# sebastianffx/stainlib

Hardware: AMD Instinct MI355X
Metric: 1024x1024 H&E tiles/sec normalized (Macenko) (higher is better)
Workload: dtype f32; 1 GPU; configs[1]: batch of 512 tiles 1024x1024x3 uint8 per GPU, Macenko transform (fit once outside the timed region), tiles resident in HBM; tiles_per_gpu=512, failed_tiles=0

## Files before the change

### stainlib_amd/csrc/stats_twosweep.hpp

```cpp
#pragma once
#include "stats_cube.hpp"

namespace sl {

constexpr double kClusterDeff = 2.0;
constexpr double kTiltZ = 5.0;
constexpr double kTiltZ4 = 4.0;
constexpr double kTsMinTau = 2e-4, kTsMaxTau = 0.05;
constexpr int kTsBackoff = 3;
constexpr double kTsAutoMaxTau = 6e-3;
constexpr int kTsMinTissue = 256;
constexpr int kTsMaxSharePct = 40;
constexpr int kTsFn = 9;
constexpr int kTsTabFloats = kTsFn * 3 * 32;

enum { kTsDirect = 1, kTsOff = 0, kTsNoEstimate = -1, kTsShare = -2, kTsPlane = -3, kTsBracket = -4, kTsLists = -5 };

struct TwoSweep {
    int ok;
    int dense;
    int pad_;
    int why;
    double Vd[6];
    double nd[3];
    double gH[3], gL[3];
    double kappa1, kappa2;
    double tau;
    float lo0, hi1;
    float fgH[3], fgL[3];
    float fn[3], fk1;
    float W[2][3], kt[2];
    float eps[2], zeta[2], thr[2];
};

struct __attribute__((packed, aligned(1))) U32U { uint32_t v; };
__device__ __forceinline__ uint32_t cluster_word(const uint8_t* src, int P, uint32_t wl, uint32_t b) {
    const uint32_t i = b / (uint32_t)kClusterPx, j = b % (uint32_t)kClusterPx;
    const uint32_t h = sample_hash(i);
    const uint32_t line = i * wl + __umulhi(h << 8, wl);
    uint32_t px = (line * 128u + 2u) / 3u + (h >> 28) % 3u + (uint32_t)kClusterStep * j;
    px = px < (uint32_t)(P - 2) ? px : (uint32_t)(P - 2);
    return ((SL_GLOBAL const U32U*)(as_global(src) + 3 * (size_t)px))->v & 0xffffffu;
}
__device__ __forceinline__ void ts_box(const double* Vd, const double* nd, double tau, const float* box, double lam, int lane, MergedConc& mk) {
    const bool finite = (box[0] > -INFINITY) & (box[1] < INFINITY) & (box[2] > -INFINITY) & (box[3] < INFINITY);
    const int g = lane % 9, var = (lane / 9) % 5;
    const int i0 = g % 3, i1 = g / 3;
    double u1[3], u2[3];
#pragma unroll
    for (int c = 0; c < 3; ++c) { u1[c] = Vd[2 * c]; u2[c] = Vd[2 * c + 1]; }
    {
        const double s = (var == 1 || var == 3) ? tau : ((var == 2 || var == 4) ? -tau : 0.0);
        const bool first = var == 1 || var == 2;
        double a[3], b[3];
#pragma unroll
        for (int c = 0; c < 3; ++c) { a[c] = (first ? u1[c] : u2[c]) + s * nd[c]; b[c] = first ? u2[c] : u1[c]; }
        const double na = 1.0 / sqrt(a[0] * a[0] + a[1] * a[1] + a[2] * a[2]);
#pragma unroll
        for (int c = 0; c < 3; ++c) a[c] *= na;
        const double ab = a[0] * b[0] + a[1] * b[1] + a[2] * b[2];
#pragma unroll
        for (int c = 0; c < 3; ++c) b[c] -= ab * a[c];
        const double nb = 1.0 / sqrt(b[0] * b[0] + b[1] * b[1] + b[2] * b[2]);
#pragma unroll
        for (int c = 0; c < 3; ++c) { b[c] *= nb; u1[c] = first ? a[c] : b[c]; u2[c] = first ? b[c] : a[c]; }
    }
    double U[6];
#pragma unroll
    for (int c = 0; c < 3; ++c) { U[2 * c] = u1[c]; U[2 * c + 1] = u2[c]; }
    const double m0 = 0.5 * ((double)box[0] + (double)box[1]), r0 = 0.5 * ((double)box[1] - (double)box[0]);
    const double m1 = 0.5 * ((double)box[2] + (double)box[3]), r1 = 0.5 * ((double)box[3] - (double)box[2]);
    const double p0 = finite ? m0 + (double)(i0 - 1) * r0 : -0.25;
    const double p1 = finite ? m1 + (double)(i1 - 1) * r1 : 0.25;
    double M[6];
    stain_matrix_from_phi(U, angle_of_pseudo(p0), angle_of_pseudo(p1), M);
    LassoD A, C;
    lasso_affine_d(M, lam, A);
#pragma unroll
    for (int i = 0; i < 2; ++i) {
#pragma unroll
        for (int c = 0; c < 3; ++c) C.W[i][c] = __shfl(A.W[i][c], 4, 64);
        C.k[i] = __shfl(A.k[i], 4, 64);
    }
    C.g12 = __shfl(A.g12, 4, 64);
    double Mc[6];
#pragma unroll
    for (int i = 0; i < 6; ++i) Mc[i] = __shfl(M[i], 4, 64);
    double T[2][2], r[2];
    relate_affine(A, C, T, r);
    double e0 = fmax(fabs(T[0][0] - 1.0), fabs(T[0][1])), e1 = fmax(fabs(T[1][1] - 1.0), fabs(T[1][0]));
    double q0 = fabs(r[0]), q1 = fabs(r[1]);
    double z0 = fabs(A.W[0][0] * nd[0] + A.W[0][1] * nd[1] + A.W[0][2] * nd[2]), z1 = fabs(A.W[1][0] * nd[0] + A.W[1][1] * nd[1] + A.W[1][2] * nd[2]);
    const bool live = lane < 45;
    const bool lane_bad = live & !((e0 <= kBoxMaxEps) & (e1 <= kBoxMaxEps) & (q0 <= 1.0) & (q1 <= 1.0) & (A.g12 >= 0.0) & (z0 <= 1.0) & (z1 <= 1.0));
    const bool any_bad = __ballot(lane_bad) != 0ull;
    if (!live || lane_bad) e0 = e1 = q0 = q1 = z0 = z1 = 0.0;
    for (int o = 32; o > 0; o >>= 1) {
        e0 = fmax(e0, __shfl_xor(e0, o, 64)); e1 = fmax(e1, __shfl_xor(e1, o, 64));
        q0 = fmax(q0, __shfl_xor(q0, o, 64)); q1 = fmax(q1, __shfl_xor(q1, o, 64));
        z0 = fmax(z0, __shfl_xor(z0, o, 64)); z1 = fmax(z1, __shfl_xor(z1, o, 64));
    }
    if (lane == 0) {
        mk.ok = (finite && !any_bad) ? 1 : 0;
        mk.pad_ = 0;
        mk.C = C;
        LassoK Lc;
        lasso_consts(Mc, lam, Lc);
        mk.Lc = Lc;
        mk.tilted = 1; mk.pad2_ = 0;
        const double e[2] = {e0, e1}, q[2] = {q0, q1}, z[2] = {z0, z1};
#pragma unroll
        for (int i = 0; i < 2; ++i) {
#pragma unroll
            for (int k = 0; k < 2; ++k) mk.u[i][k] = (float)(C.W[i][0] * Vd[k] + C.W[i][1] * Vd[2 + k] + C.W[i][2] * Vd[4 + k]);
            mk.kt[i] = (float)C.k[i];
            mk.eta[i] = 4e-6 * (kOdMax * (fabs(C.W[i][0]) + fabs(C.W[i][1]) + fabs(C.W[i][2])) + fabs(C.k[i]) + 1.0);
            mk.eps[i] = (float)(kBoxInflate * e[i] + 1e-7);
            mk.rho[i] = kBoxInflate * q[i] + mk.eta[i];
            mk.zeta[i] = kBoxInflate * z[i] + 1e-7;
            mk.nrm[i] = nd[i];
        }
        mk.nrm[2] = nd[2];
    }
}
__device__ __forceinline__ void ts_thresholds(MergedConc& mk, float lo0, float lo1, float hi0, float hi1, float zref) {
    const float lo[2] = {lo0, lo1}, hi[2] = {hi0, hi1};
    bool ok = mk.ok != 0;
    float ref[2];
#pragma unroll
    for (int i = 0; i < 2; ++i) ref[i] = hi[i] < INFINITY ? hi[i] : 2.0f * lo[i] + 1.0f;
#pragma unroll
    for (int i = 0; i < 2; ++i) {
        const float delta = mk.eps[i] * (ref[i] + 1.5f * ref[1 - i]) + (float)mk.rho[i] + (float)mk.zeta[i] * zref;
        mk.L[i] = lo[i] - delta;
        mk.H[i] = hi[i] + delta;
        ok = ok & (mk.L[i] > 0.0f) & (lo[i] > -INFINITY);
        mk.thr[i] = mk.L[i] - (float)mk.rho[i] - 1e-6f * fabsf(mk.L[i]);
    }
    if (!ok) {
        mk.ok = 0;
#pragma unroll
        for (int i = 0; i < 2; ++i) { mk.u[i][0] = mk.u[i][1] = mk.kt[i] = mk.eps[i] = 0.0f; mk.thr[i] = INFINITY; mk.L[i] = mk.H[i] = INFINITY; mk.zeta[i] = 0.0; }
    }
}

struct TsCubeConsts { float k1, s_ang, kt[2], eps[2], zeta[2], thr[2]; };
__device__ __forceinline__ TsCubeConsts ts_cube_tables(const TabView& tab, const TwoSweep& ts, float* ctab, int tid) {
    TsCubeConsts cc;
    cc.k1 = ts.fk1;
    float sg = 0.0f;
    for (int c = 0; c < 3; ++c) sg = fmaxf(sg, fmaxf(fabsf(ts.fgH[c]), fabsf(ts.fgL[c])));
    float sn = fabsf(ts.fn[0]) + fabsf(ts.fn[1]) + fabsf(ts.fn[2]);
    cc.s_ang = 8e-6f * ((float)kOdMax * (3.0f * sg + ts.fk1 * sn) + 1.0f);
#pragma unroll
    for (int i = 0; i < 2; ++i) {
        cc.kt[i] = ts.kt[i]; cc.eps[i] = ts.eps[i]; cc.zeta[i] = ts.zeta[i];
        const float ca = fabsf(ts.W[i][0]) + fabsf(ts.W[i][1]) + fabsf(ts.W[i][2]);
        cc.thr[i] = ts.thr[i] - 8e-6f * ((float)kOdMax * (ca * (1.0f + 2.0f * ts.eps[i]) + ts.zeta[i] * sn) + fabsf(ts.kt[i]) + 1.0f);
    }
    for (int e = tid; e < kTsTabFloats; e += (int)blockDim.x) {
        const int f = e / 96, ch = (e / 32) % 3, k = e & 31;
        const float od_lo = tab.odf((uint32_t)(8 * k + 7)), od_hi = tab.odf((uint32_t)(8 * k));
        float out;
        if (f == 0) {
            const float w = ch == 0 ? 871.0f : (ch == 1 ? 2929.0f : 296.0f);
            out = w * tab.gam((uint32_t)(8 * k));
        } else {
            float c;
            switch (f) {
                case 1: c = ts.fgH[ch]; break;
                case 2: c = ts.fgL[ch]; break;
                case 3: case 4: c = ts.fn[ch]; break;
                case 5: case 6: c = ts.W[0][ch]; break;
                default: c = ts.W[1][ch]; break;
            }
            const bool want_max = (f == 4) | (f == 6) | (f == 8);
            const float a = c * od_lo, b = c * od_hi;
            out = want_max ? fmaxf(a, b) : fminf(a, b);
        }
        ctab[e] = out;
    }
    return cc;
}
__device__ __forceinline__ bool ts_cell_verdict(const float* v, const TsCubeConsts& cc, float ylimf) {
    const bool no_tissue = v[0] >= ylimf;
    const float zabs = fmaxf(fabsf(v[3]), fabsf(v[4]));
    const bool cone = fmaf(-cc.k1, zabs, fminf(v[1], v[2])) > cc.s_ang;
    const float sa = fmaxf(fabsf(v[5]), fabsf(v[6])) + fmaxf(fabsf(v[7]), fabsf(v[8]));
    const bool conc1 = fmaf(cc.zeta[0], zabs, fmaf(cc.eps[0], sa, v[6])) < cc.thr[0], conc2 = fmaf(cc.zeta[1], zabs, fmaf(cc.eps[1], sa, v[8])) < cc.thr[1];
    return (no_tissue || cone) && conc1 && conc2;
}
__device__ __forceinline__ bool ts_cell_plain(const float* ctab, const TsCubeConsts& cc, float ylimf, uint32_t p) {
    const int r5 = (int)((p >> 3) & 31u), g5 = (int)((p >> 11) & 31u), b5 = (int)((p >> 19) & 31u);
    float v[kTsFn];
#pragma unroll
    for (int f = 0; f < kTsFn; ++f)
        v[f] = ctab[(f * 3 + 1) * 32 + g5] + ctab[(f * 3 + 2) * 32 + b5] + (f >= 5 ? cc.kt[(f - 5) >> 1] : 0.0f) + ctab[(f * 3) * 32 + r5];
    return ts_cell_verdict(v, cc, ylimf);
}
template <int NT>
__device__ __forceinline__ void ts_cube_mask(const float* ctab, const TsCubeConsts& cc, float ylimf, uint32_t* bits, int tid) {
    for (int w = tid; w < kCubeWords; w += NT) {
        const int g5 = w & 31, b5 = w >> 5;
        float part[kTsFn];
#pragma unroll
        for (int f = 0; f < kTsFn; ++f) part[f] = ctab[(f * 3 + 1) * 32 + g5] + ctab[(f * 3 + 2) * 32 + b5] + (f >= 5 ? cc.kt[(f - 5) >> 1] : 0.0f);
        uint32_t word = 0;
        for (int r5 = 0; r5 < 32; ++r5) {
            float v[kTsFn];
#pragma unroll
            for (int f = 0; f < kTsFn; ++f) v[f] = part[f] + ctab[(f * 3) * 32 + r5];
            word |= ts_cell_verdict(v, cc, ylimf) ? 0u : (1u << r5);
        }
        bits[w] = word;
    }
}
template <int NT>
__device__ __forceinline__ int ts_cube_share(const uint32_t* samp, int n_sample, const float* ctab, const TsCubeConsts& cc, float ylimf, unsigned int* counter, int tid) {
    if (tid == 0) *counter = 0;
    __syncthreads();
    uint32_t amb = 0, seen = 0;
    for (int b = tid; b < n_sample; b += kCubeShareStep * NT) {
        amb += ts_cell_plain(ctab, cc, ylimf, as_global(samp)[b] & 0xffffffu) ? 0u : 1u;
        ++seen;
    }
    uint32_t both = amb | (seen << 16);
    for (int o = 32; o > 0; o >>= 1) both += (uint32_t)__shfl_xor((int)both, o, 64);
    if ((tid & 63) == 0 && both) atomicAdd(counter, both);
    __syncthreads();
    const uint32_t tot = *counter;
    return (tot >> 16) ? (int)(100u * (tot & 0xffffu) / (tot >> 16)) : 100;
}

struct TsSweepConsts {
    float gH[3], gL[3], n[3], k1;
    float W[2][3], kt[2], eps[2], zeta[2], thr[2];
};
template <bool ALIGNED, int kTrip, bool STREAM>
__device__ __forceinline__ void ts_sweep(const uint8_t* src, int P, int c0, int c1, int t, int nthreads, const TabReaderB& T, float ylimf,
                                         const TsSweepConsts& K, uint32_t bits_lds, uint32_t ring_lds, const RawDirect& out, Moments& mo,
                                         uint32_t& n_tissue) {
    const size_t nbytes = (size_t)P * 3;
    const int lane = t & 63;
    const int w0 = __builtin_amdgcn_readfirstlane(c0 + (t & ~63));
    using G = GatherGamOd;
    auto fetch = [&](int cc) { return load_chunk_clamped<ALIGNED, STREAM>(src, nbytes, cc, c1); };
    auto gather = [&](const Chunk& ch) { return gather_gam_od(T, ch); };
    BurstMoments bm;
    auto compute = [&](auto tail_tag, const G& g, int cc) {
        constexpr bool TAIL = decltype(tail_tag)::value;
#pragma unroll
        for (int px = 0; px < 4; ++px) {
            const float2 er = g.v[3 * px], eg = g.v[3 * px + 1], eb = g.v[3 * px + 2];
            const bool tc = is_tissue_f(er.x, eg.x, eb.x, ylimf);
            const bool ok = tc & (!TAIL || in_tile<ALIGNED>(cc, px, c1, P));
#if defined(__HIP_DEVICE_COMPILE__)
            unsigned long long carry;
            asm("v_addc_co_u32 %0, %1, 0, %0, %2" : "+v"(n_tissue), "=s"(carry) : "s"(__builtin_amdgcn_ballot_w64(ok)));
#else
            n_tissue += ok ? 1u : 0u;
#endif
            if (ok) bm.add(er.y, eg.y, eb.y);
        }
    };
    CubeRing ring = CubeRing::make(ring_lds);
    struct G3 { float2 r, g, b; };
    auto gather3 = [&](uint32_t q) { return G3{T.gam_odf(T.addr(q, 0)), T.gam_odf(T.addr(q, 1)), T.gam_odf(T.addr(q, 2))}; };
    struct M2 { unsigned long long a, c; };
    auto flags = [&](const G3& e) -> M2 {
        const bool tc = is_tissue_f(e.r.x, e.g.x, e.b.x, ylimf);
        const float z = fmaf(K.n[2], e.b.y, fmaf(K.n[1], e.g.y, K.n[0] * e.r.y));
        const float tH = fmaf(K.gH[2], e.b.y, fmaf(K.gH[1], e.g.y, K.gH[0] * e.r.y));
        const float tL = fmaf(K.gL[2], e.b.y, fmaf(K.gL[1], e.g.y, K.gL[0] * e.r.y));
        const bool pp = fmaf(-K.k1, fabsf(z), fminf(tH, tL)) > 0.0f;
        const float a1 = fmaf(K.W[0][2], e.b.y, fmaf(K.W[0][1], e.g.y, fmaf(K.W[0][0], e.r.y, K.kt[0])));
        const float a2 = fmaf(K.W[1][2], e.b.y, fmaf(K.W[1][1], e.g.y, fmaf(K.W[1][0], e.r.y, K.kt[1])));
        const float sa = fabsf(a1) + fabsf(a2);
        const bool g1 = fmaf(K.zeta[0], fabsf(z), fmaf(K.eps[0], sa, a1)) >= K.thr[0], g2 = fmaf(K.zeta[1], fabsf(z), fmaf(K.eps[1], sa, a2)) >= K.thr[1];
        return M2{__builtin_amdgcn_ballot_w64(tc) & ~__builtin_amdgcn_ballot_w64(pp), __builtin_amdgcn_ballot_w64(g1) | __builtin_amdgcn_ballot_w64(g2)};
    };
    auto drain = [&]() {
        while (ring.two_rows()) {
            uint32_t q0, q1;
            ring.pop2(lane, q0, q1);
            const G3 e0 = gather3(q0), e1 = gather3(q1);
            const M2 f0 = flags(e0), f1 = flags(e1);
            out.put2(f0.a, f0.c, q0, f1.a, f1.c, q1, lane);
        }
    };
    auto cube = [&](auto tail_tag, const Chunk& ch, int cc) {
        constexpr bool TAIL = decltype(tail_tag)::value;
        uint32_t p[4];
        bool amb[4];
#pragma unroll
        for (int px = 0; px < 4; ++px) {
            p[px] = chunk_pixel(ch, px);
            amb[px] = cube_ambiguous(px == 0 ? ch.w0 : p[px], bits_lds);
        }
#pragma unroll
        for (int px = 0; px < 4; px += 2) {
            unsigned long long m[2];
#pragma unroll
            for (int j = 0; j < 2; ++j) {
                m[j] = __builtin_amdgcn_ballot_w64(amb[px + j]);
                if (TAIL) m[j] &= __builtin_amdgcn_ballot_w64(in_tile<ALIGNED>(cc, px + j, c1, P));
            }
            ring.put2(m[0], p[px] & 0xffffffu, m[1], p[px + 1] & 0xffffffu);
            drain();
        }
    };
    Chunk cur[kTrip], nx[kTrip];
#pragma unroll
    for (int k = 0; k < kTrip; ++k) { cur[k] = fetch(w0 + lane + k * nthreads); nx[k] = fetch(w0 + lane + (kTrip + k) * nthreads); }
    auto trip = [&](auto tail_tag, int cb) {
        G g[2];
        g[0] = gather(cur[0]);
#pragma unroll
        for (int k = 0; k < kTrip; ++k) cube(tail_tag, cur[k], cb + k * nthreads + lane);
#pragma unroll
        for (int k = 0; k < kTrip; ++k) {
            if (k + 1 < kTrip) {
                g[(k + 1) & 1] = gather(cur[k + 1]);
            } else {
#pragma unroll
                for (int j = 0; j < kTrip; ++j) { cur[j] = nx[j]; nx[j] = fetch(cb + lane + (2 * kTrip + j) * nthreads); }
            }
            __builtin_amdgcn_sched_barrier(0);
            compute(tail_tag, g[k & 1], cb + k * nthreads + lane);
            __builtin_amdgcn_sched_barrier(0);
        }
        bm.flush(mo);
    };
    const int lim = ALIGNED ? c1 : min(c1, P >> 2);
    int cb = w0;
    for (; cb + (kTrip - 1) * nthreads + 64 <= lim; cb += nthreads * kTrip) trip(std::false_type{}, cb);
    if (cb < c1) trip(std::true_type{}, cb);
    {
        uint32_t q0, q1;
        ring.rest2(lane, q0, q1);
        const uint32_t rn = ring.fill();
        const G3 e0 = gather3(q0 & 0xffffffu), e1 = gather3(q1 & 0xffffffu);
        const unsigned long long l0 = __builtin_amdgcn_ballot_w64((uint32_t)lane < rn), l1 = __builtin_amdgcn_ballot_w64(64u + (uint32_t)lane < rn);
        const M2 f0 = flags(e0), f1 = flags(e1);
        out.put2(f0.a & l0, f0.c & l0, q0, f1.a & l1, f1.c & l1, q1, lane);
    }
}

__device__ __forceinline__ bool ts_verify(const TwoSweep& ts, const double* Vd, float* br , int lane, bool force_fail) {
    double n[3] = {Vd[2] * Vd[5] - Vd[4] * Vd[3], Vd[4] * Vd[1] - Vd[0] * Vd[5], Vd[0] * Vd[3] - Vd[2] * Vd[1]};
    const double nn = 1.0 / sqrt(n[0] * n[0] + n[1] * n[1] + n[2] * n[2]);
    const double sgn = (n[0] * ts.nd[0] + n[1] * ts.nd[1] + n[2] * ts.nd[2]) < 0.0 ? -nn : nn;
    double dn = 0.0;
#pragma unroll
    for (int c = 0; c < 3; ++c) { n[c] *= sgn; dn = fmax(dn, fabs(n[c] - ts.nd[c])); }
    const double cH = fabs(n[0] * ts.gH[0] + n[1] * ts.gH[1] + n[2] * ts.gH[2]), cL = fabs(n[0] * ts.gL[0] + n[1] * ts.gL[1] + n[2] * ts.gL[2]);
    const double cmax = fmax(cH, cL);
    bool ok = (cmax <= ts.kappa1) & (cmax * dn <= ts.kappa2) & !force_fail;
    const double qH[2] = {Vd[0] * ts.gH[0] + Vd[2] * ts.gH[1] + Vd[4] * ts.gH[2], Vd[1] * ts.gH[0] + Vd[3] * ts.gH[1] + Vd[5] * ts.gH[2]};
    const double qL[2] = {Vd[0] * ts.gL[0] + Vd[2] * ts.gL[1] + Vd[4] * ts.gL[2], Vd[1] * ts.gL[0] + Vd[3] * ts.gL[1] + Vd[5] * ts.gL[2]};
    const double rHx = qH[1], rHy = -qH[0], rLx = -qL[1], rLy = qL[0];
    ok = ok & (rHx > 1e-3) & (rLx > 1e-3);
    const double pH = rHy / (fabs(rHx) + fabs(rHy)), pL = rLy / (fabs(rLx) + fabs(rLy));
    ok = ok & (pH + 4.0 * (double)kAngleMargin < pL);
    const double pad = 4.0 * ts.tau + 1e-3;
    double ends[2] = {(double)ts.lo0, (double)ts.hi1};
#pragma unroll
    for (int e = 0; e < 2; ++e) {
        const double p = ends[e];
        if (p > -1.0 && p < 1.0) {
            const double dx = 1.0 - fabs(p), dy = p;
            double v3[3];
#pragma unroll
            for (int c = 0; c < 3; ++c) v3[c] = ts.Vd[2 * c] * dx + ts.Vd[2 * c + 1] * dy;
            const double x = Vd[0] * v3[0] + Vd[2] * v3[1] + Vd[4] * v3[2], y = Vd[1] * v3[0] + Vd[3] * v3[1] + Vd[5] * v3[2];
            ends[e] = x > 0.0 ? y / (x + fabs(y)) + (e == 0 ? -pad : pad) : (e == 0 ? -INFINITY : INFINITY);
        } else {
            ends[e] = e == 0 ? -INFINITY : INFINITY;
        }
    }
    br[0] = (float)ends[0];
    br[1] = (float)pH - kAngleMargin;
    br[2] = (float)pL + kAngleMargin;
    br[3] = (float)ends[1];
    if (!(br[0] < br[1])) br[0] = -INFINITY;
    if (!(br[3] > br[2])) br[3] = INFINITY;
    (void)lane;
    return ok;
}

}
```

### stainlib_amd/csrc/sweep_pipeline.hpp

```cpp
#pragma once
#include "apply_kernels.hpp"
#include <type_traits>

namespace sl {

template <bool ALIGNED>
__device__ __forceinline__ bool in_tile(int cc, int px, int c1, int P) {
    return (cc < c1) & (ALIGNED | ((size_t)cc * 4 + px < (size_t)P));
}

struct GatherGamOd { float2 v[12]; };
struct GatherOd { float v[12]; };
template <class TR>
__device__ __forceinline__ GatherGamOd gather_gam_od(const TR& T, const Chunk& ch) {
    GatherGamOd g;
#pragma unroll
    for (int i = 0; i < 12; ++i) g.v[i] = T.gam_odf(T.addr(ch, i));
    return g;
}
template <class TR>
__device__ __forceinline__ GatherOd gather_od(const TR& T, const Chunk& ch) {
    GatherOd g;
#pragma unroll
    for (int i = 0; i < 12; ++i) g.v[i] = T.odf(T.addr(ch, i));
    return g;
}

template <bool ALIGNED, int kTrip, bool STREAM, class Gather, class Compute>
__device__ __forceinline__ void pipelined_sweep(const uint8_t* src, int P, int c0, int c1, int t, int nthreads,
                                                Gather gather, Compute compute) {
    const size_t nbytes = (size_t)P * 3;
    const int lane = t & 63;
    const int w0 = __builtin_amdgcn_readfirstlane(c0 + (t & ~63));
    auto fetch = [&](int cc) { return load_chunk_clamped<ALIGNED, STREAM>(src, nbytes, cc, c1); };
    Chunk cur[kTrip], nx[kTrip];
#pragma unroll
    for (int k = 0; k < kTrip; ++k) { cur[k] = fetch(w0 + lane + k * nthreads); nx[k] = fetch(w0 + lane + (kTrip + k) * nthreads); }
    decltype(gather(cur[0])) g[2];
    g[0] = gather(cur[0]);
    auto trip = [&](auto tail_tag, int cb) {
#pragma unroll
        for (int k = 0; k < kTrip; ++k) {
            const Chunk ch = cur[k];
            if (k + 1 < kTrip) {
                g[(k + 1) & 1] = gather(cur[k + 1]);
            } else {
#pragma unroll
                for (int j = 0; j < kTrip; ++j) { cur[j] = nx[j]; nx[j] = fetch(cb + lane + (2 * kTrip + j) * nthreads); }
                g[0] = gather(cur[0]);
            }
            __builtin_amdgcn_sched_barrier(0);
            compute(tail_tag, ch, g[k & 1], cb + k * nthreads + lane);
            __builtin_amdgcn_sched_barrier(0);
        }
    };
    const int lim = ALIGNED ? c1 : min(c1, P >> 2);
    int cb = w0;
    for (; cb + (kTrip - 1) * nthreads + 64 <= lim; cb += nthreads * kTrip) trip(std::false_type{}, cb);
    if (cb < c1) trip(std::true_type{}, cb);
}

}
```

Measured before the change: 381,700 tiles/s.

## Replace two-sweep loop with ping-pong lookahead sweep that refetches per slot

The stats two-sweep loop now uses a new generic lookahead_wave_sweep helper. It alternates between two chunk buffers (X/Y), and each slot is refetched right after it has been gathered, instead of copying the whole next buffer at the end of a trip. Clamping moves into the helper, and an empty asm barrier pins the moments in registers after each flush. The goal is to spread global loads more evenly across the trip and cut register copies. The cost is more scheduling barriers and a loop unrolled across two trips, which may raise register pressure.

```diff
diff --git a/stainlib_amd/csrc/stats_twosweep.hpp b/stainlib_amd/csrc/stats_twosweep.hpp
--- a/stainlib_amd/csrc/stats_twosweep.hpp
+++ b/stainlib_amd/csrc/stats_twosweep.hpp
@@ -244,7 +244,7 @@
     const int lane = t & 63;
     const int w0 = __builtin_amdgcn_readfirstlane(c0 + (t & ~63));
     using G = GatherGamOd;
-    auto fetch = [&](int cc) { return load_chunk_clamped<ALIGNED, STREAM>(src, nbytes, cc, c1); };
+    auto fetch = [&](int cc) { return load_chunk<ALIGNED, STREAM>(src, nbytes, cc); };
     auto gather = [&](const Chunk& ch) { return gather_gam_od(T, ch); };
     BurstMoments bm;
     auto compute = [&](auto tail_tag, const G& g, int cc) {
@@ -309,32 +309,13 @@
             drain();
         }
     };
-    Chunk cur[kTrip], nx[kTrip];
-#pragma unroll
-    for (int k = 0; k < kTrip; ++k) { cur[k] = fetch(w0 + lane + k * nthreads); nx[k] = fetch(w0 + lane + (kTrip + k) * nthreads); }
-    auto trip = [&](auto tail_tag, int cb) {
-        G g[2];
-        g[0] = gather(cur[0]);
-#pragma unroll
-        for (int k = 0; k < kTrip; ++k) cube(tail_tag, cur[k], cb + k * nthreads + lane);
-#pragma unroll
-        for (int k = 0; k < kTrip; ++k) {
-            if (k + 1 < kTrip) {
-                g[(k + 1) & 1] = gather(cur[k + 1]);
-            } else {
-#pragma unroll
-                for (int j = 0; j < kTrip; ++j) { cur[j] = nx[j]; nx[j] = fetch(cb + lane + (2 * kTrip + j) * nthreads); }
-            }
-            __builtin_amdgcn_sched_barrier(0);
-            compute(tail_tag, g[k & 1], cb + k * nthreads + lane);
-            __builtin_amdgcn_sched_barrier(0);
-        }
+    auto end_trip = [&]() {
         bm.flush(mo);
-    };
-    const int lim = ALIGNED ? c1 : min(c1, P >> 2);
-    int cb = w0;
-    for (; cb + (kTrip - 1) * nthreads + 64 <= lim; cb += nthreads * kTrip) trip(std::false_type{}, cb);
-    if (cb < c1) trip(std::true_type{}, cb);
+#if defined(__HIP_DEVICE_COMPILE__)
+        asm volatile("" : "+v"(mo.sx), "+v"(mo.sy), "+v"(mo.sz), "+v"(mo.sxx), "+v"(mo.sxy), "+v"(mo.sxz), "+v"(mo.syy), "+v"(mo.syz), "+v"(mo.szz));
+#endif
+    };
+    lookahead_wave_sweep<kTrip>(w0, lane, c1, ALIGNED ? c1 : min(c1, P >> 2), nthreads, fetch, gather, cube, compute, end_trip);
     {
         uint32_t q0, q1;
         ring.rest2(lane, q0, q1);
diff --git a/stainlib_amd/csrc/sweep_lookahead.hpp b/stainlib_amd/csrc/sweep_lookahead.hpp
--- /dev/null
+++ b/stainlib_amd/csrc/sweep_lookahead.hpp
@@ -0,0 +1,58 @@
+#pragma once
+#include <type_traits>
+
+#if defined(__HIPCC__)
+#define SL_LOOKAHEAD_FN __host__ __device__ __forceinline__
+#else
+#define SL_LOOKAHEAD_FN inline
+#endif
+#if defined(__HIP_DEVICE_COMPILE__)
+#define SL_LOOKAHEAD_FENCE() __builtin_amdgcn_sched_barrier(0)
+#else
+#define SL_LOOKAHEAD_FENCE() ((void)0)
+#endif
+
+namespace sl {
+
+template <int N, class FETCH, class GATHER, class HEAD, class COMPUTE, class ENDTRIP>
+SL_LOOKAHEAD_FN void lookahead_wave_sweep(int w0, int lane, int c1, int lim, int nthreads, const FETCH& fetch, const GATHER& gather,
+                                          const HEAD& head, const COMPUTE& compute, const ENDTRIP& end_trip) {
+    using CH = decltype(fetch(0));
+    auto fetch_clamped = [&](int c) { return fetch(c < c1 ? c : c1 - 1); };
+    CH X[N], Y[N];
+#pragma unroll
+    for (int k = 0; k < N; ++k) { X[k] = fetch_clamped(w0 + lane + k * nthreads); SL_LOOKAHEAD_FENCE(); }
+#pragma unroll
+    for (int k = 0; k < N; ++k) { Y[k] = fetch_clamped(w0 + lane + (N + k) * nthreads); SL_LOOKAHEAD_FENCE(); }
+    auto trip = [&](auto tail_tag, CH (&cur)[N], int cb) {
+        decltype(gather(cur[0])) g[2];
+        g[0] = gather(cur[0]);
+#pragma unroll
+        for (int k = 0; k < N; ++k) head(tail_tag, cur[k], cb + k * nthreads + lane);
+        cur[0] = fetch_clamped(cb + lane + 2 * N * nthreads);
+#pragma unroll
+        for (int k = 0; k < N; ++k) {
+            if (k + 1 < N) {
+                g[(k + 1) & 1] = gather(cur[k + 1]);
+                cur[k + 1] = fetch_clamped(cb + lane + (2 * N + k + 1) * nthreads);
+            }
+            SL_LOOKAHEAD_FENCE();
+            compute(tail_tag, g[k & 1], cb + k * nthreads + lane);
+            SL_LOOKAHEAD_FENCE();
+        }
+        end_trip();
+        SL_LOOKAHEAD_FENCE();
+    };
+    const int step = N * nthreads;
+    int cb = w0;
+    for (; cb + (2 * N - 1) * nthreads + 64 <= lim; cb += 2 * step) {
+        trip(std::false_type{}, X, cb);
+        trip(std::false_type{}, Y, cb + step);
+    }
+    if (cb < c1) {
+        trip(std::true_type{}, X, cb);
+        if (cb + step < c1) trip(std::true_type{}, Y, cb + step);
+    }
+}
+
+}
diff --git a/stainlib_amd/csrc/sweep_pipeline.hpp b/stainlib_amd/csrc/sweep_pipeline.hpp
--- a/stainlib_amd/csrc/sweep_pipeline.hpp
+++ b/stainlib_amd/csrc/sweep_pipeline.hpp
@@ -1,5 +1,6 @@
 #pragma once
 #include "apply_kernels.hpp"
+#include "sweep_lookahead.hpp"
 #include <type_traits>
 
 namespace sl {
```

New measurement: 387,000 tiles/s (median of 6 runs). 1.4% higher.
